# SAIC-MONTREAL/multimodal-dynamics

Hardware: AMD Instinct MI355X
Metric: visuotactile samples/sec (train) + ELBO vs CPU ref, cnn-mvae 64x64 bs256 @1/2/4/8 GPU (higher is better)
Workload: dtype f32x3; 1 GPU; cnn-mvae visuotactile+pose 64x64, bs=256 per GPU, fp32 storage and results, GEMMs in the fp32x3 arithmetic (exact three-term bf16 split of the fp32 operands, six of nine products on the bf16 matrix cores, fp32 accumulate; error vs fp64 <= native fp32 MFMA), seq_modeling train step (7 subset ELBOs + backward + Adam), BASELINE configs[1]; global_batch=256, parallelism=dp1, bn=local, launch=hip_graph

## Files before the change

include/mmdyn_hip.h:

```cpp
#ifndef MMDYN_HIP_H
#define MMDYN_HIP_H

#include <stdint.h>

#ifdef __cplusplus
extern "C" {
#endif

#define MMDYN_OK 0
#define MMDYN_ERR_SHAPE (-1)
#define MMDYN_ERR_NULL (-2)
#define MMDYN_ERR_RANGE (-3)

#define MMDYN_ACT_NONE 0
#define MMDYN_ACT_SWISH 1
#define MMDYN_ACT_RELU 2

#define MMDYN_DENSE 0
#define MMDYN_CONV 1
#define MMDYN_TCONV_S2P1 2
#define MMDYN_IM2COL3 3

#define MMDYN_TCONV_S1P0 4

// ... 273 lines not shown

int mmdyn_sgd_step(float* p, const float* g, float* momentum_buf, int64_t n, float lr, float momentum,
                   float weight_decay, float grad_scale, int first, void* stream);

int mmdyn_resize_ksize(int in_size, int out_size);
int mmdyn_resize_plan(int in_size, int out_size, int* bounds, int* coeffs);
int mmdyn_resize_u8_to_chw_f32(const uint8_t* src, const int* index, float* dst, int n_out, int Hin, int Win,
                               int Hout, int Wout, const int* xb, const int* xk, const int* yb, const int* yk,
                               void* stream);

int mmdyn_igemm_nt_mx(const void* A, const void* Bp, const float* bias, void* C, void* C_act, float* stats,
                      float* ws, const void* y, const float* mean, const float* rstd, const float* gamma,
                      const float* beta, int mode, int G, int Bg, int Hi, int Wi, int Cin, int Ho, int Wo, int N,
                      int ldc, int stride, int offset, int act, int splitk, int flags, uint32_t* arrival_flags, void* stream);
int mmdyn_wgrad_tn_mx(const void* D, const void* Gt, float* partial, int mode, int Bt, int Hr, int Wr, int Cd, int Hi,
                      int Wi, int Cg, int stride, int offset, int chunks, int flags, void* stream);
int mmdyn_split_planes(const float* x, void* planes, int64_t rows, int C, void* stream);
int mmdyn_igemm_planes_served(int mode, int G, int Bg, int Hi, int Wi, int Cin, int Ho, int Wo, int N);
int mmdyn_bn_swish_fwd_planes(const float* y, const float* mean, const float* rstd, const float* gamma, const float* beta,
                              float* a, void* a_planes, int G, int rows_per_group, int C, void* stream);
int mmdyn_bn_swish_bwd_apply_planes(const float* da, const float* y, const float* mean, const float* rstd, const float* gamma,
                                    const float* beta, const float* sums, float* dy, void* dy_planes, int G, int rows_per_group,
                                    int C, int da_is_du, void* stream);
int mmdyn_bn_eval_swish_bwd(const float* da, const float* y, const float* mean, const float* rstd, const float* gamma,
                            const float* beta, float* dy, void* dy_planes, float* partial, int G, int rows_per_group, int C,
                            int da_is_du, void* stream);
int mmdyn_bn_swish_fwd_b16(const uint16_t* y, const float* mean, const float* rstd, const float* gamma,
                           const float* beta, uint16_t* a, int G, int rows_per_group, int C, int half, void* stream);
int mmdyn_bn_swish_bwd_reduce_b16(const uint16_t* da, const uint16_t* y, const float* mean, const float* rstd,
                                  const float* gamma, const float* beta, float* partial, int G, int rows_per_group,
                                  int C, int half, void* stream);
int mmdyn_bn_swish_bwd_apply_b16(const uint16_t* da, const uint16_t* y, const float* mean, const float* rstd,
                                 const float* gamma, const float* beta, const float* sums, uint16_t* dy, int G,
                                 int rows_per_group, int C, int da_is_du, int half, void* stream);
int mmdyn_act_bwd_b16(const uint16_t* dh, const uint16_t* u, uint16_t* du, int64_t n, int act, int half, void* stream);
int mmdyn_tconv_out3_fwd_b16(const uint16_t* a, const float* w, float* out, int Bt, int Hi, int Wi, int half,
                             void* stream);

int mmdyn_nchw_to_nhwc(const float* in, float* out, int B, int C, int HW, void* stream);
int mmdyn_nhwc_to_nchw(const float* in, float* out, int B, int C, int HW, void* stream);

int mmdyn_concat_condition(const float* x, const float* cond, const int64_t* cond_idx, float* out, int* bad_index, int rows,
                           int K, int ldx, int cd, int width, void* stream);
int mmdyn_concat_condition_tiled(const float* x, const float* cond, const int64_t* cond_idx, float* out, int* bad_index, int rows,
                                 int x_rows, int K, int ldx, int cd, int width, void* stream);

// ... 5 lines not shown
```

multimodal-dynamics_amd/csrc/bn.hip:

```cpp
#include "common.h"

namespace {

static int tile_rows_for(int rows_per_group) {
  int t = rows_per_group / 256 / 32 * 32;
  return t < 32 ? 32 : (t > 512 ? 512 : t);
}

struct BnParams {
  const float* mean;
  const float* rstd;
  const float* gamma;
  const float* beta;
};

template <int MODE, typename TA>
__global__ __launch_bounds__(256) void colreduce_kernel(const TA* __restrict__ y,
                                                        const TA* __restrict__ da, BnParams bp,
                                                        float* __restrict__ partial, int rows_per_group,
                                                        int C, int T, int tile_rows) {
  __shared__ float red[256 * 8];
  const int tid = threadIdx.x;
  const int g = blockIdx.y, t = blockIdx.x;
  const int CV = C >> 2;
// ... 331 lines not shown
  for (int64_t i = blockIdx.x * (int64_t)blockDim.x + threadIdx.x; i < total8; i += (int64_t)gridDim.x * blockDim.x) {
    const int cv = (int)(i % CV);
    const int64_t row = i / CV;
    const int g = (int)(row / rows_per_group);
    f32x4 v[2], d[2], o[2];
    ldv_nt<float>(y + i * 8, v);
    ldv_nt<float>(y + i * 8 + 4, v + 1);
    ldv_nt<float>(da + i * 8, d);
    ldv_nt<float>(da + i * 8 + 4, d + 1);
#pragma unroll
    for (int q = 0; q < 2; ++q) {
      const int c0 = cv * 8 + q * 4;
      f32x4 m = *reinterpret_cast<const f32x4*>(bp.mean + (size_t)g * C + c0);
      f32x4 r = *reinterpret_cast<const f32x4*>(bp.rstd + (size_t)g * C + c0);
      f32x4 ga = *reinterpret_cast<const f32x4*>(bp.gamma + c0);
      f32x4 be = *reinterpret_cast<const f32x4*>(bp.beta + c0);
      f32x4 s0 = *reinterpret_cast<const f32x4*>(sums + ((size_t)g * 2 + 0) * C + c0);
      f32x4 s1 = *reinterpret_cast<const f32x4*>(sums + ((size_t)g * 2 + 1) * C + c0);
#pragma unroll
      for (int k = 0; k < 4; ++k) {
        float xh = (v[q][k] - m[k]) * r[k];
        float u = ga[k] * xh + be[k];
        float du = da_is_du ? d[q][k] : d[q][k] * swish_gradf_(u);
        o[q][k] = ga[k] * r[k] * (du - s0[k] * inv_n - xh * (s1[k] * inv_n));
      }
    }
    if (dy) {
      stv_nt<float>(dy + i * 8, o);
      stv_nt<float>(dy + i * 8 + 4, o + 1);
    }
    store_planes8(dyp + row * 3 * (int64_t)C + cv * 8, C, o[0], o[1]);
  }
}

template <bool NEED_Y, bool PARTIAL>
__global__ __launch_bounds__(256) void bn_eval_swish_bwd_kernel(const float* __restrict__ da, const float* __restrict__ y, BnParams bp,
                                                                float* __restrict__ dy, bf16_t* __restrict__ dyp,
                                                                float* __restrict__ partial, int rows_per_group, int C, int T,
                                                                int tile_rows, int da_is_du) {
  __shared__ float red[PARTIAL ? 256 * 16 : 1];
  const int tid = threadIdx.x;
  const int g = blockIdx.y, t = blockIdx.x;
  const int CV = C >> 3;
  const int RL = 256 / CV;
  const int rl = tid / CV, cv = tid - rl * CV;
  const int r_begin = t * tile_rows;
  const int r_end = min(rows_per_group, r_begin + tile_rows);
// ... 323 lines not shown
```

multimodal-dynamics_amd/csrc/common.h:

```cpp
#pragma once
#include <hip/hip_runtime.h>
#include <stdint.h>
#include <stdlib.h>
#include "mmdyn_hip.h"

typedef float f32x16 __attribute__((ext_vector_type(16)));
typedef float f32x4 __attribute__((ext_vector_type(4)));

typedef uint16_t bf16_t;
template <typename T> __device__ __forceinline__ f32x4 ld4(const T* p);
template <> __device__ __forceinline__ f32x4 ld4<float>(const float* p) { return *reinterpret_cast<const f32x4*>(p); }
template <> __device__ __forceinline__ f32x4 ld4<bf16_t>(const bf16_t* p) {
  const uint2 u = *reinterpret_cast<const uint2*>(p);
  f32x4 v;
  v[0] = __uint_as_float(u.x << 16);
  v[1] = __uint_as_float(u.x & 0xffff0000u);
  v[2] = __uint_as_float(u.y << 16);
  v[3] = __uint_as_float(u.y & 0xffff0000u);
  return v;
}
template <typename T> __device__ __forceinline__ float ld1(const T* p);
template <> __device__ __forceinline__ float ld1<float>(const float* p) { return *p; }
template <> __device__ __forceinline__ float ld1<bf16_t>(const bf16_t* p) { return __uint_as_float((uint32_t)*p << 16); }
__device__ __forceinline__ uint32_t pack2_bf16(float lo, float hi) {
// ... 228 lines not shown
  return v;
}

__device__ __forceinline__ void block_atomic_add(double v, double* dst, double scale = 1.0) {
  v = wave_sum_d(v);
  __shared__ double red[4];
  if ((threadIdx.x & 63) == 0) red[threadIdx.x >> 6] = v;
  __syncthreads();
  if (threadIdx.x == 0) atomicAdd(dst, scale * (red[0] + red[1] + red[2] + red[3]));
}

constexpr float POE_EPS = 1e-8f;

constexpr uint32_t ALL_PRESENT = 0x01010101u;
__device__ __forceinline__ bool has(uint32_t word, int m) { return ((word >> (8 * m)) & 0xffu) != 0u; }

__device__ __forceinline__ float sigmoid_exact(float v) { return 1.f / (1.f + expf(-v)); }
__device__ __forceinline__ float sigmoidf_(float x) { return __builtin_amdgcn_rcpf(1.0f + __expf(-x)); }
__device__ __forceinline__ float swishf_(float x) { return x * sigmoidf_(x); }
__device__ __forceinline__ float swish_gradf_(float x) {
  float s = sigmoidf_(x);
  return s * (1.0f + x * (1.0f - s));
}
__device__ __forceinline__ float apply_act(float x, int act) {
  if (act == MMDYN_ACT_SWISH) return swishf_(x);
  if (act == MMDYN_ACT_RELU) return x > 0.f ? x : 0.f;
  return x;
}
__device__ __forceinline__ float act_grad(float x, int act) {
  if (act == MMDYN_ACT_SWISH) return swish_gradf_(x);
  if (act == MMDYN_ACT_RELU) return x > 0.f ? 1.f : 0.f;
  return 1.f;
}

__device__ __forceinline__ void bce_elem(float x, float t, float& loss, float& sig) {
  const float e = __expf(-fabsf(x));
  const float inv = __frcp_rn(__fadd_rn(1.f, e));
  loss = __fadd_rn(__fsub_rn(fmaxf(x, 0.f), __fmul_rn(x, t)), __logf(__fadd_rn(1.f, e)));
  sig = x >= 0.f ? inv : __fmul_rn(e, inv);
}

int mmdyn_conv3_nt_try(const float* A, const float* Bp, const float* bias, void* C, void* C_act, float* stats, int G,
                       int Bg, int Hi, int Wi, int Ho, int Wo, int N, int ldc, int act, int splitk, const void* bn_y,
                       const float* bn_mean, const float* bn_rstd, const float* bn_gamma, const float* bn_beta,
                       int c_b16, int bny_b16, int b_b16, hipStream_t st);
int mmdyn_conv3_wgrad_try(const void* D, const float* Gt, float* partial, int Bt, int Hr, int Wr, int Cd, int Hi,
// ... 25 lines not shown
```

multimodal-dynamics_amd/csrc/conv3.hip:

```cpp
#include "common.h"

namespace {

struct Conv3Geom {
  int G, Bg, Hi, Wi, Ho, ldc;
  int act, want_act_out, want_stats, w_b16;
  int tiles_per_group;
  const void* bn_y;
  const float* bn_mean;
  const float* bn_rstd;
  const float* bn_gamma;
  const float* bn_beta;
};

#define GLOBAL_AS __attribute__((address_space(1)))
typedef GLOBAL_AS char* gchar_p;
__device__ __forceinline__ gchar_p sgpr_ptr(const void* p) {
  const uint64_t u = reinterpret_cast<uint64_t>(p);
  const uint32_t lo = __builtin_amdgcn_readfirstlane((uint32_t)u), hi = __builtin_amdgcn_readfirstlane((uint32_t)(u >> 32));
  return (gchar_p)(((uint64_t)hi << 32) | lo);
}
template <typename T> __device__ __forceinline__ float gld1(gchar_p p);
template <> __device__ __forceinline__ float gld1<float>(gchar_p p) { return *(GLOBAL_AS const float*)p; }
template <> __device__ __forceinline__ float gld1<bf16_t>(gchar_p p) {
  return __uint_as_float((uint32_t)(*(GLOBAL_AS const bf16_t*)p) << 16);
}
template <> __device__ __forceinline__ float gld1<half_t>(gchar_p p) { return h2f(*(GLOBAL_AS const uint16_t*)p); }
template <typename T> struct store16 { typedef bf16_t type; };
template <> struct store16<half_t> { typedef half_t type; };

constexpr int C3_N = 32;
template <typename T, bool BN, int ACT, int SEGS>
__global__ __launch_bounds__(256) __attribute__((amdgpu_waves_per_eu(4, 4))) void conv3_nt_kernel(
    const float* __restrict__ img, const float* __restrict__ Wp, T* __restrict__ C, T* __restrict__ C_act,
    float* __restrict__ stats, const Conv3Geom g) {
  __shared__ float Ws[32 * 65];
  __shared__ float red[4][2][32];
  const int tid = threadIdx.x, lane = tid & 63;
  const int wave = __builtin_amdgcn_readfirstlane(tid >> 6);
  const int x = lane & 31, h = lane >> 5;
  for (int i = tid; i < 512; i += 256) {
    const f32x4 v = g.w_b16 == 2 ? ld4<half_t>(reinterpret_cast<const half_t*>(Wp) + 4 * i)
                    : g.w_b16 ? ld4<bf16_t>(reinterpret_cast<const bf16_t*>(Wp) + 4 * i)
                              : reinterpret_cast<const f32x4*>(Wp)[i];
    const int n = i >> 4, k = (i & 15) * 4;
    Ws[n * 65 + k + 0] = v[0];
    Ws[n * 65 + k + 1] = v[1];
    Ws[n * 65 + k + 2] = v[2];
    Ws[n * 65 + k + 3] = v[3];
  }
  __syncthreads();
  float bw[24];
  auto load_bw = [&]() {
#pragma unroll
    for (int j = 0; j < 24; ++j) bw[j] = Ws[x * 65 + (j >> 3) * 16 + ((j >> 1) & 3) * 4 + 2 * (j & 1) + h];
  };
  if (!BN) load_bw();

  const float bn_g = BN ? g.bn_gamma[x] : 0.f, bn_b = BN ? g.bn_beta[x] : 0.f;
  const int ntiles = g.G * g.tiles_per_group;

  constexpr int C3_HI = 64 * SEGS, C3_HO = 32 * SEGS;
  constexpr int UNITS = C3_HO * SEGS;
  int xl[2];
#pragma unroll
  for (int q = 0; q < 2; ++q) xl[q] = 2 * x - 1 + 2 * q + h;
  const unsigned voffB = (4 * h * C3_N + x) * sizeof(T);
  constexpr unsigned IMG_B = 3 * C3_HI * C3_HI * sizeof(float);
  constexpr unsigned OROW_B = 32 * C3_N * sizeof(T);

  struct TileAt {
    gchar_p imgb;
    size_t orow;
    int y, seg;
    unsigned xoB[2];
    bool xok[2];
  };
  auto locate = [&](int t) {
    TileAt p;
    const int u = t * 4 + wave;
    const int ib = u / UNITS, rem = u - ib * UNITS;
    p.y = rem / SEGS;
    p.seg = rem - p.y * SEGS;
    p.imgb = sgpr_ptr(reinterpret_cast<const char*>(img) + (size_t)ib * IMG_B + (size_t)p.seg * 256 - 4);
    p.orow = (size_t)u * OROW_B;
#pragma unroll
    for (int q = 0; q < 2; ++q) {
      p.xok[q] = (unsigned)(p.seg * 64 + xl[q]) < (unsigned)C3_HI;
      p.xoB[q] = (unsigned)((p.xok[q] ? xl[q] + 1 : 1) * 4);
    }
    return p;
  };
  auto load_a = [&](const TileAt& p, int j) {
    const int ci = j >> 3, yin = 2 * p.y - 1 + ((j >> 1) & 3);
    const bool yok = (unsigned)yin < (unsigned)C3_HI;
    const gchar_p rowp = p.imgb + (unsigned)((ci * C3_HI + (yok ? yin : 0)) * C3_HI) * 4u;
    return gld1<float>(rowp + p.xoB[j & 1]);
  };
  auto erow = [](int e) { return (unsigned)(((e & 3) + 8 * (e >> 2)) * C3_N * sizeof(T)); };

  float a[24], yv[16];
  int t = blockIdx.x;
  if (t >= ntiles) return;
  TileAt cur = locate(t);
#pragma unroll
  for (int j = 0; j < 24; ++j) a[j] = load_a(cur, j);
  if (BN) {
    const gchar_p yb = sgpr_ptr(reinterpret_cast<const char*>(g.bn_y) + cur.orow) + voffB;
#pragma unroll
    for (int e = 0; e < 16; ++e) yv[e] = gld1<T>(yb + erow(e));
  }
  for (; t < ntiles; t += gridDim.x) {
    const int tn = t + gridDim.x < ntiles ? t + gridDim.x : t;
    const TileAt nxt = locate(tn);
    const int grp = (BN || g.want_stats) ? __builtin_amdgcn_readfirstlane((t / (UNITS / 4)) / g.Bg) : 0;
    if (BN) load_bw();
    float bn_m = 0.f, bn_r = 0.f;
    if (BN) {
      bn_m = g.bn_mean[grp * 32 + x];
      bn_r = g.bn_rstd[grp * 32 + x];
    }
    f32x16 acc;
#pragma unroll
    for (int e = 0; e < 16; ++e) acc[e] = 0.f;
#pragma unroll
    for (int j = 0; j < 24; ++j) {
      const int yin = 2 * cur.y - 1 + ((j >> 1) & 3);
      const bool ok = ((unsigned)yin < (unsigned)C3_HI) & cur.xok[j & 1];
      acc = __builtin_amdgcn_mfma_f32_32x32x2f32(ok ? a[j] : 0.f, bw[j], acc, 0, 0, 0);
      a[j] = load_a(nxt, j);
    }

    const gchar_p cb = sgpr_ptr(reinterpret_cast<const char*>(C) + cur.orow) + voffB;
    const gchar_p ab = sgpr_ptr(reinterpret_cast<const char*>(C_act) + cur.orow) + voffB;
    const gchar_p yb = sgpr_ptr(reinterpret_cast<const char*>(g.bn_y) + nxt.orow) + voffB;
    float cs = 0.f, cq = 0.f;
#pragma unroll
    for (int e = 0; e < 16; ++e) {
      float v = acc[e];
      if (BN) {
        const float xh = (yv[e] - bn_m) * bn_r;
        yv[e] = gld1<T>(yb + erow(e));
        v *= swish_gradf_(bn_g * xh + bn_b);
        cs += v;
        cq += v * xh;
      } else {
        cs += v;
        cq += v * v;
      }
      if (sizeof(T) == 2) {
        const float vn = __shfl_down(v, 1, 64);
        if (!(x & 1)) {
          *(GLOBAL_AS uint32_t*)(cb + erow(e)) = pack2<typename store16<T>::type>(v, vn);
          if (ACT >= 0)
            *(GLOBAL_AS uint32_t*)(ab + erow(e)) = pack2<typename store16<T>::type>(apply_act(v, ACT), apply_act(vn, ACT));
        }
      } else {
        *(GLOBAL_AS float*)(cb + erow(e)) = v;
        if (ACT >= 0) *(GLOBAL_AS float*)(ab + erow(e)) = apply_act(v, ACT);
      }
    }
    if (g.want_stats) {
      cs += __shfl_xor(cs, 32, 64);
      cq += __shfl_xor(cq, 32, 64);
      if (h == 0) {
        red[wave][0][x] = cs;
        red[wave][1][x] = cq;
      }
      __syncthreads();
      if (tid < 32) {
        float s0 = 0.f, q0 = 0.f;
#pragma unroll
        for (int w = 0; w < 4; ++w) {
// ... 192 lines not shown
      if (segs == 1) CONV3_LAUNCH(half_t, BN_, ACT_, 1);                                                           \
      else if (segs == 2) CONV3_LAUNCH(half_t, BN_, ACT_, 2);                                                      \
      else CONV3_LAUNCH(half_t, BN_, ACT_, 4);                                                                     \
    } else if (c_b16) {                                                                                            \
      if (segs == 1) CONV3_LAUNCH(bf16_t, BN_, ACT_, 1);                                                           \
      else if (segs == 2) CONV3_LAUNCH(bf16_t, BN_, ACT_, 2);                                                      \
      else CONV3_LAUNCH(bf16_t, BN_, ACT_, 4);                                                                     \
    } else {                                                                                                       \
      if (segs == 1) CONV3_LAUNCH(float, BN_, ACT_, 1);                                                            \
      else if (segs == 2) CONV3_LAUNCH(float, BN_, ACT_, 2);                                                       \
      else CONV3_LAUNCH(float, BN_, ACT_, 4);                                                                      \
    }                                                                                                              \
  }
  CONV3_CASE(4, true, -1)
  CONV3_CASE(-1, false, -1)
  CONV3_CASE(MMDYN_ACT_NONE, false, MMDYN_ACT_NONE)
  CONV3_CASE(MMDYN_ACT_SWISH, false, MMDYN_ACT_SWISH)
  CONV3_CASE(MMDYN_ACT_RELU, false, MMDYN_ACT_RELU)
#undef CONV3_LAUNCH
#undef CONV3_CASE
  MMDYN_LAUNCH_CHECK();
}

int mmdyn_conv3_wgrad_try(const void* D, const float* Gt, float* partial, int Bt, int Hr, int Wr, int Cd, int Hi,
                          int Wi, int Cg, int chunks, int d_b16, hipStream_t st, const float* bn_mean, const float* bn_rstd,
                          const float* bn_gamma, const float* bn_beta, int Bg) {
  if (Cd != 32 || Cg != 64 || Wr != Hr || Wi != Hi || Hi != 2 * Hr || (Hi != 64 && Hi != 128 && Hi != 256)) return 1;
  const int segs = Hi / 64;
  if ((int64_t)Bt * Hr * segs >= (1LL << 30)) return 1;
  Conv3WgradGeom g{};
  g.Bt = Bt;
  g.Hr = Hr;
  g.Hi = Hi;
  g.Wi = Wi;
  g.img_rows = Bt * Hr * segs;
  g.rows_per_chunk = ceil_div(g.img_rows, chunks);
  g.bn_mean = bn_mean;
  g.bn_rstd = bn_rstd;
  g.bn_gamma = bn_gamma;
  g.bn_beta = bn_beta;
  g.Bg = Bg > 0 ? Bg : Bt;
#define CONV3_WG(T_, S_)                                                                                                  \
  do {                                                                                                                    \
    if (bn_mean)                                                                                                          \
      hipLaunchKernelGGL((conv3_wgrad_kernel<T_, S_, true>), dim3(chunks), dim3(256), 0, st, (const T_*)D, Gt, partial, g); \
    else                                                                                                                  \
// ... 19 lines not shown
```

multimodal-dynamics_amd/mmdyn_hip/_lib.py:

```python
import ctypes
import os

_HERE = os.path.dirname(os.path.abspath(__file__))
LIB_PATH = os.environ.get("MMDYN_HIP_LIB") or os.path.join(_HERE, "libmmdyn_hip.so")

_P, _I, _L, _F, _Q = ctypes.c_void_p, ctypes.c_int, ctypes.c_int64, ctypes.c_float, ctypes.c_uint64


class PassExperts(ctypes.Structure):
    _fields_ = [("mu", _P * 4), ("lv", _P * 4), ("dmu", _P * 4), ("dlv", _P * 4), ("ld", _I * 4), ("dz", _P * 3),
                ("zdst", _P * 3), ("zpl", _P * 3)]


class PackEntry(ctypes.Structure):
    _fields_ = [("src", _P), ("dst", _P), ("kind", _I), ("rows_in", _I), ("cols_in", _I), ("rows_out", _I),
                ("cols_out", _I), ("ld_out", _I), ("dst_bf16", _I)]


class FeedGroups(ctypes.Structure):
    _fields_ = [("recon", _P * 4), ("obs", _P * 4), ("out", _P * 4), ("row_len", _I * 4), ("logits", _I * 4), ("column", _I * 4)]


class GatherGroups(ctypes.Structure):
    _fields_ = [("src", _P * 4), ("out", _P * 4), ("row_len", _I * 4), ("logits", _I * 4)]
# ... 68 lines not shown
    "mmdyn_cast_f32_to_bf16": "pp" + "l" + "p",
    "mmdyn_cast_bf16_to_f32": "pp" + "l" + "p",
    "mmdyn_linear_small_fwd": "pppp" + "iiii" + "p",
    "mmdyn_linear_small_bwd": "pppppp" + "iii" + "f" + "p",
    "mmdyn_poe_fwd": "pppppp" + "iiii" + "p",
    "mmdyn_poe_bwd": "ppppppp" + "f" + "iiii" + "pp",
    "mmdyn_reparam_fwd": "ppppp" + "iii" + "p",
    "mmdyn_reparam_bwd": "pppp" + "f" + "pp" + "iii" + "p",
    "mmdyn_bce_logits": "ppppp" + "l" + "iii" + "f" + "p",
    "mmdyn_bce_logits_groups": "ppppp" + "i" + "l" + "f" + "p",
    "mmdyn_bce_logits_groups_masked": "ppppppp" + "i" + "l" + "iii" + "f" + "p",
    "mmdyn_mse": "pppp" + "l" + "f" + "p",
    "mmdyn_mse_groups": "ppppp" + "i" + "l" + "f" + "p",
    "mmdyn_elbo_assemble": "ppppp" + "ii" + "ff" + "pp",
    "mmdyn_adam_step": "ppppp" + "l" + "fffff" + "p",
    "mmdyn_adam_step_guarded": "ppppp" + "l" + "fffff" + "p",
    "mmdyn_sgd_step": "ppp" + "l" + "ffff" + "i" + "p",
    "mmdyn_igemm_nt_mx": "pppppppppppp" + "iiiiiiiiiiiiii" + "i" + "pp",
    "mmdyn_wgrad_tn_mx": "ppp" + "iiiiiiiiiii" + "i" + "p",
    "mmdyn_split_planes": "pp" + "l" + "i" + "p",
    "mmdyn_igemm_planes_served": "iiiiiiiii",
    "mmdyn_bn_swish_fwd_planes": "ppppppp" + "iii" + "p",
    "mmdyn_bn_swish_bwd_apply_planes": "ppppppppp" + "iiii" + "p",
    "mmdyn_bn_eval_swish_bwd": "ppppppppp" + "iiii" + "p",
    "mmdyn_bn_swish_fwd_b16": "pppppp" + "iiii" + "p",
    "mmdyn_bn_swish_bwd_reduce_b16": "ppppppp" + "iiii" + "p",
    "mmdyn_bn_swish_bwd_apply_b16": "pppppppp" + "iiiii" + "p",
    "mmdyn_act_bwd_b16": "ppp" + "l" + "ii" + "p",
    "mmdyn_tconv_out3_fwd_b16": "ppp" + "iiii" + "p",
    "mmdyn_resize_ksize": "ii",
    "mmdyn_resize_plan": "ii" + "pp",
    "mmdyn_resize_u8_to_chw_f32": "ppp" + "iiiii" + "pppp" + "p",
    "mmdyn_nchw_to_nhwc": "pp" + "iii" + "p",
    "mmdyn_nhwc_to_nchw": "pp" + "iii" + "p",
    "mmdyn_tconv_out3_bn_bce_rows": "ppppppp" + "i" + "pp" + "i" + "ppp" + "iiiiii" + "p",
    "mmdyn_bce_logits_rows_groups": "ppp" + "i" + "ppp" + "iiiii" + "p",
    "mmdyn_mse_rows_groups": "pppp" + "iiii" + "p",
    "mmdyn_kl_rows": "ppp" + "iii" + "p",
    "mmdyn_elbo_assemble_rows": "pppppp" + "ii" + "ff" + "p" + "i" + "p",
    "mmdyn_concat_condition": "ppppp" + "iiiii" + "p",
    "mmdyn_poe_fwd_avail": "ppppppp" + "iiii" + "p",
    "mmdyn_poe_bwd_avail": "pppppppp" + "f" + "iiii" + "pp",
    "mmdyn_complete_select": "ppp" + "i" + "p" + "iii" + "p",
    "mmdyn_elbo_assemble_rows_avail": "ppppppppp" + "ii" + "ff" + "p" + "i" + "p",
    "mmdyn_tconv_out3_bn_bce_rows_grad": "ppppppp" + "i" + "pp" + "i" + "ppppp" + "i" + "f" + "iiiii" + "p",
    "mmdyn_bce_logits_rows_groups_grad": "ppp" + "i" + "ppppp" + "i" + "f" + "iiii" + "p",
# ... 61 lines not shown
```

multimodal-dynamics_amd/mmdyn_hip/layers.py:

```python
import weakref

import torch

from . import ops
from .ops import ACT_NONE, ACT_SWISH, ACT_RELU, DENSE, CONV, TCONV_S2P1, IM2COL3, TCONV_S1P0
from .models.shapes import BN_EPS, BN_MOMENTUM, FEAT


def _new(like, *shape, dtype=torch.float32):
    if isinstance(like, ops.Planes):
        like = like.t
    return torch.empty(shape, device=like.device, dtype=dtype)


ACT_DTYPE = torch.float32
W_DTYPE = torch.float32


def _act(like, *shape):
    return torch.empty(shape, device=like.device, dtype=ACT_DTYPE)


def _cdiv(a, b):
    return (a + b - 1) // b
# ... 31 lines not shown
        ops.B.igemm_nt(A, Bp, None, C, None, None, ws, DENSE, 1, rows, 1, 1, K, 1, 1, N, N, 1, 0, ACT_NONE, splitk)
        ops.B.splitk_reduce(ws, bias, C, Ca, splitk, rows, N, act)
    else:
        ops.B.igemm_nt(A, Bp, bias, C, Ca, None, None, DENSE, 1, rows, 1, 1, K, 1, 1, N, N, 1, 0, act, 1)
    return C, Ca


PLANES = True
PLANE_TWIN = {}


def _plane_twin(Wp):
    ent = PLANE_TWIN.get(Wp.data_ptr())
    if ent is None:
        return None
    if ent[0]() is not Wp:
        if ent[0]() is None:
            del PLANE_TWIN[Wp.data_ptr()]
        return None
    return ent[1]


PATCH_PLANES = True


def planes_served(mode, G, Bg, Hi, Cin, Ho, N):
    served = getattr(ops.B, "igemm_planes_served", None) if PLANES else None
    if N == 32 and not PATCH_PLANES:
        return False
    return bool(served is not None and ACT_DTYPE == torch.float32 and served(mode, G, Bg, Hi, Hi, Cin, Ho, Ho, N))


def split_operands(x, Wp, mode, G, Bg, Hi, Cin, Ho, N):
    if isinstance(Wp, ops.Planes):
        return x, Wp
    xin = x.t if isinstance(x, ops.Planes) else x
    if xin.dtype not in (torch.float32, torch.bfloat16) or Wp.dtype != torch.float32 or not planes_served(mode, G, Bg, Hi, Cin, Ho, N):
        if isinstance(x, ops.Planes):
            raise ValueError("mmdyn_hip: a plane operand for a launch the plane-ring kernel does not serve")
        return x, Wp
    if not isinstance(x, ops.Planes):
        xp = ops.Planes(x.numel() // Cin, Cin, x.device)
        ops.B.split_planes(x, xp)
        x = xp
    wp = _plane_twin(Wp)
    if wp is None or wp.C != Cin or wp.rows * Cin != Wp.numel():
# ... 177 lines not shown
        ops.backend_op("bn_eval_swish_bwd")(da, y, mean, rstd, bn.gamma, bn.beta, dy, partial, G, rows_per_group, C, False, planes=dyp)
        if partial is not None:
            _bn_eval_param_grads(y, partial, T, dgamma, dbeta, G, C)
        return dy if dyp is None else dyp
    partial = _new(y, G, T, 2, C)
    ops.B.bn_swish_bwd_reduce(da, y, mean, rstd, bn.gamma, bn.beta, partial, G, rows_per_group, C)
    sums = _bn_backward_sums(y, partial, T, dgamma, dbeta, G, C)
    dy, dyp = _apply_out(y, planes_out)
    if dyp is not None:
        ops.B.bn_swish_bwd_apply(da, y, mean, rstd, bn.gamma, bn.beta, sums, None, G, rows_per_group, C, planes=dyp)
        return dyp
    ops.B.bn_swish_bwd_apply(da, y, mean, rstd, bn.gamma, bn.beta, sums, dy, G, rows_per_group, C)
    return dy


def dgrad_bn_swish_backward(x, Wp, mode, G, Bg, Hi, Cin, Ho, N, stride, offset, y, mean, rstd, bn, dgamma, dbeta, planes_out=False,
                            eval_mode=False):
    rows_per_group = Bg * Ho * Ho
    if eval_mode:
        _eval_mode_check()
    if y.dtype == torch.float32 and mode != IM2COL3:
        x, Wp = split_operands(x, Wp, mode, G, Bg, Hi, Cin, Ho, N)
    T = _stat_tiles(x, Wp, mode, G, Bg, Hi, Cin, Ho, N)
    du = torch.empty_like(y)
    partial = _new(y, G, T, 2, N)
    ops.B.igemm_nt_dgrad_bn(x, Wp, du, partial, y, mean, rstd, bn.gamma, bn.beta, mode, G, Bg, Hi, Hi, Cin, Ho, Ho, N,
                            stride, offset)
    if eval_mode:
        if dgamma is not None or dbeta is not None:
            _bn_eval_param_grads(y, partial, T, dgamma, dbeta, G, N)
        dy, dyp = _apply_out(y, planes_out)
        ops.backend_op("bn_eval_swish_bwd")(du, None, mean, rstd, bn.gamma, bn.beta, dy, None, G, rows_per_group, N, True, planes=dyp)
        return dy if dyp is None else dyp
    sums = _bn_backward_sums(y, partial, T, dgamma, dbeta, G, N)
    dy, dyp = _apply_out(y, planes_out)
    if dyp is not None:
        ops.B.bn_swish_bwd_apply(du, y, mean, rstd, bn.gamma, bn.beta, sums, None, G, rows_per_group, N, True, planes=dyp)
        return dyp
    ops.B.bn_swish_bwd_apply(du, y, mean, rstd, bn.gamma, bn.beta, sums, dy, G, rows_per_group, N, True)
    return dy


def wgrad(D, Gt, canon, mode, Bt, Hr, Cd, Hi, Cg, stride=1, offset=0, cg_canon=None, perm=0, defer=None):
    if defer is not None:
        defer.append((D, Gt, canon, mode, Bt, Hr, Cd, Hi, Cg, stride, offset, cg_canon, perm))
        return
    rows = Bt * Hr * Hr
    taps = 16 if mode == CONV else 1
# ... 347 lines not shown
            with ctx():
                try:
                    next(gen)
                except StopIteration as e:
                    results[i] = e.value
                    live.remove(i)
    return results


def encoder_trunk_forward(*a, **k):
    return run(encoder_trunk_forward_steps(*a, **k))


def encoder_trunk_forward_steps(P, buf, x, G=1, repeat=1, packed=None, training=True):
    Bt = x.shape[0]
    Bg = Bt // G
    convs, S = enc_layout(P)
    if tuple(x.shape[1:]) != (3, S, S):
        raise ValueError(f"mmdyn_hip: this encoder takes [B,3,{S},{S}] images, got {tuple(x.shape)}")
    pk = packed if packed is not None else pack_now(encoder_pack_specs(P))
    c = {"Bt": Bt, "G": G, "Bg": Bg, "pk": pk, "S": S, "training": bool(training)}
    H = S // 2
    W1p = pk["W1p"]
    u1, a1 = _act(x, Bt * H * H, 32), _act(x, Bt * H * H, 32)
    ops.B.igemm_nt(x, W1p, None, u1, a1, None, None, IM2COL3, 1, Bt, S, S, 64, H, H, 32, 32, 1, 0,
                   ACT_SWISH, 1)
    yield
    stages, a, cin = [], a1, 32
    if len(convs) and planes_served(CONV, G, Bg, H, 32, H // 2, P[f"conv_net.{convs[0]}.weight"].shape[0]):
        a = as_planes(a1, 32)
    for j, i in enumerate(convs):
        cout = P[f"conv_net.{i}.weight"].shape[0]
        last = j == len(convs) - 1
        Ho, stride, offset = (H - 3, 1, 0) if last else (H // 2, 2, -1)
        bn = _bn_of(P, buf, f"conv_net.{i + 1}")
        y, st, T = conv_like(a, pk[f"W{j + 2}k"], CONV, G, Bg, H, cin, Ho, cout, stride, offset, training)
        want = False
        if not last:
            nlast = j + 1 == len(convs) - 1
            want = planes_served(CONV, G, Bg, Ho, cout, Ho - 3 if nlast else Ho // 2, P[f"conv_net.{convs[j + 1]}.weight"].shape[0])
        an, m, r = bn_swish_from_partials(y, st, T, bn, G, Bg * Ho * Ho, cout, repeat, planes=want)
        stages.append(dict(i=i, Hi=H, Ho=Ho, cin=cin, cout=cout, stride=stride, offset=offset, a_in=a, y=y, a=an, m=m, r=r,
                           bn=bn))
        a, cin, H = an, cout, Ho
        yield
    u5, h = dense(a, pk["Wf"], P["fc_net.0.bias"], Bt, FEAT, 512, ACT_SWISH, want_act=True)
    c.update(x=x, u1=u1, a1=a1, u5=u5, stages=stages)
    return h, c


def encoder_trunk_backward(*a, **k):
    return run(encoder_trunk_backward_steps(*a, **k))
# ... 306 lines not shown
```

multimodal-dynamics_amd/mmdyn_hip/ops.py:

```python
import ctypes

import os

import torch

from . import _lib
from ._lib import PassExperts, FeedGroups, GatherGroups, EnsembleGroups, MAX_PASSES, MAX_EXPERTS, FEED_GROUPS, check

ACT_NONE, ACT_SWISH, ACT_RELU = 0, 1, 2
DENSE, CONV, TCONV_S2P1, IM2COL3, TCONV_S1P0 = 0, 1, 2, 3, 4
ROW_GROUPS_MAX = 8
PLAN_TOP_MAX = 8
REFIT_N_MAX = 4096


def _ptr(t, dtype=torch.float32):
    if t is None:
        return None
    if not t.is_cuda:
        raise RuntimeError("mmdyn_hip: the HIP path needs GPU tensors (got a CPU tensor); there is no CPU fallback")
    if t.dtype != dtype:
        raise TypeError(f"mmdyn_hip: expected {dtype}, got {t.dtype}")
    if not t.is_contiguous():
        raise ValueError("mmdyn_hip: tensor must be contiguous")
# ... 534 lines not shown
    def bn_bwd_finalize_sums(self, sums, sums_f, dgamma, dbeta, G, C, sums_scale, beta_acc):
        check(self.lib.mmdyn_bn_bwd_finalize_sums(_ptr(sums, torch.float64), _ptr(sums_f), _ptr(dgamma), _ptr(dbeta), G, C,
                                                  float(sums_scale), float(beta_acc), _stream()),
              "mmdyn_bn_bwd_finalize_sums")

    def bn_swish_bwd_apply(self, da, y, mean, rstd, gamma, beta, sums, dy, G, rows_per_group, C, da_is_du=False, planes=None):
        if planes is not None:
            if planes.rows != G * rows_per_group or planes.C != C:
                raise ValueError("mmdyn_hip: bn_swish_bwd_apply: plane tensor of the wrong shape")
            check(self.lib.mmdyn_bn_swish_bwd_apply_planes(_ptr(da), _ptr(y), _ptr(mean), _ptr(rstd), _ptr(gamma), _ptr(beta), _ptr(sums),
                                                           _ptr(dy), planes.t.data_ptr(), G, rows_per_group, C, int(da_is_du), _stream()),
                  "mmdyn_bn_swish_bwd_apply_planes")
            return
        (pd, d16), (py, y16), (po, o16) = _aptr(da), _aptr(y), _aptr(dy)
        if not (d16 == y16 == o16):
            raise TypeError("mmdyn_hip: bn_swish_bwd_apply tensors must share the storage type")
        if y16:
            check(self.lib.mmdyn_bn_swish_bwd_apply_b16(pd, py, _ptr(mean), _ptr(rstd), _ptr(gamma), _ptr(beta), _ptr(sums), po,
                                                        G, rows_per_group, C, int(da_is_du), _half(y16), _stream()),
                  "mmdyn_bn_swish_bwd_apply_b16")
            return
        check(self.lib.mmdyn_bn_swish_bwd_apply(pd, py, _ptr(mean), _ptr(rstd), _ptr(gamma), _ptr(beta), _ptr(sums), po, G,
                                                rows_per_group, C, int(da_is_du), _stream()), "mmdyn_bn_swish_bwd_apply")

    def bn_eval_swish_bwd(self, da, y, mean, rstd, gamma, beta, dy, partial, G, rows_per_group, C, da_is_du=False, planes=None):
        if planes is not None and (planes.rows != G * rows_per_group or planes.C != C):
            raise ValueError("mmdyn_hip: bn_eval_swish_bwd: plane tensor of the wrong shape")
        n = G * rows_per_group * C
        for t in (da, y, dy):
            if t is not None and t.numel() != n:
                raise ValueError("mmdyn_hip: bn_eval_swish_bwd: da / y / dy must hold G * rows_per_group * C elements")
        if partial is not None and partial.numel() != G * self.colstats_tiles(rows_per_group) * 2 * C:
            raise ValueError("mmdyn_hip: bn_eval_swish_bwd: partial must be [G][colstats_tiles(rows_per_group)][2][C]")
        if mean.numel() != G * C or rstd.numel() != G * C or gamma.numel() != C or beta.numel() != C:
            raise ValueError("mmdyn_hip: bn_eval_swish_bwd: mean / rstd are [G][C], gamma / beta [C]")
        check(self.lib.mmdyn_bn_eval_swish_bwd(_ptr(da), _ptr(y), _ptr(mean), _ptr(rstd), _ptr(gamma), _ptr(beta), _ptr(dy),
                                               None if planes is None else planes.t.data_ptr(), _ptr(partial), G, rows_per_group, C,
                                               int(da_is_du), _stream()), "mmdyn_bn_eval_swish_bwd")

    def act_fwd(self, u, h, act):
        check(self.lib.mmdyn_act_fwd(_ptr(u), _ptr(h), u.numel(), act, _stream()), "mmdyn_act_fwd")

    def act_bwd(self, dh, u, du, act):
        (pd, d16), (pu, u16), (po, o16) = _aptr(dh), _aptr(u), _aptr(du)
        if not (d16 == u16 == o16):
            raise TypeError("mmdyn_hip: act_bwd tensors must share the storage type")
# ... 694 lines not shown
```

multimodal-dynamics_amd/mmdyn_hip/profiling.py:

```python
import collections

import torch

from . import ops

PAD_CYCLES = 100000
HOST_ONLY = {"igemm_stat_tiles", "colstats_tiles", "wgrad_chunks", "igemm_planes_served"}


def _canon(name, a):
    if name == "igemm_nt_dgrad_bn":
        A, Bp, C, stats, y, mean, rstd, gamma, beta, mode, G, Bg, Hi, Wi, Cin, Ho, Wo, N, stride, offset = a
        name, a = "igemm_nt", (A, Bp, y, C, None, stats, None, mode, G, Bg, Hi, Wi, Cin, Ho, Wo, N, N, stride, offset, 0, 1)
    if name == "igemm_nt_dgrad_act":
        A, Bp, C, u, act, mode, G, Bg, Hi, Wi, Cin, Ho, Wo, N, stride, offset = a
        name, a = "igemm_nt", (A, Bp, u, C, None, None, None, mode, G, Bg, Hi, Wi, Cin, Ho, Wo, N, N, stride, offset, 0, 1)
    if name == "igemm_nt_grouped":
        A, Bp, bias, C, C_act, u, G, rows, K, N, act = a
        name, a = "igemm_nt", (A, Bp, bias if u is None else u, C, C_act, None, None, ops.DENSE, G, rows, 1, 1, K, 1, 1, N, N, 1, 0, act, 1)
    if name == "wgrad_tn_grouped":
        D, Gt, partial, G, rows, Cd, Cg, chunks = a
        name, a = "wgrad_tn", (D, Gt, partial, ops.DENSE, G * rows, 1, 1, Cd, 1, 1, Cg, 1, 0, chunks)
    if name == "wgrad_out3_bn":
        y, mean, rstd, gamma, beta, Gt, partial, G, Bg, Hr, chunks = a
        return "conv3_wgrad", (y, Gt, partial, ops.IM2COL3, G * Bg, Hr, Hr, 32, 2 * Hr, 2 * Hr, 64, 1, 0, chunks)
    if name == "tconv_out3_bn_fwd":
        return "tconv_out3_fwd", a
    if name == "igemm_nt" and a[7] == ops.IM2COL3 and a[10] in (64, 128, 256) and \
            tuple(a[10:17]) == (a[10], a[10], 64, a[10] // 2, a[10] // 2, 32, 32):
        return "conv3_nt", a
    if name == "igemm_nt" and a[7] == ops.TCONV_S2P1 and tuple(a[10:16]) in ((16, 16, 64, 32, 32, 32), (32, 32, 32, 64, 64, 32),
                                                                            (64, 64, 32, 128, 128, 32)) and \
            getattr(ops.B, "precision", "fp32") == "fp32" and all(not torch.is_tensor(t) or t.dtype == torch.float32 for t in a[:4]):
        return "tconv_patch", a
    if name == "wgrad_tn" and a[3] == ops.IM2COL3 and a[8] in (64, 128, 256) and \
            tuple(a[5:11]) == (a[8] // 2, a[8] // 2, 32, a[8], a[8], 64):
        return "conv3_wgrad", a
    return name, a


def _flops(name, a):
    if name in ("igemm_nt", "conv3_nt", "tconv_patch"):
        (mode, G, Bg, Hi, Wi, Cin, Ho, Wo, N) = a[7:16]
        if mode == ops.DENSE:
            return 2.0 * G * Bg * Ho * Wo * N * Cin
        if mode == ops.CONV:
            return 2.0 * G * Bg * Ho * Wo * N * 16 * Cin
        if mode == ops.TCONV_S1P0:
            return 2.0 * G * Bg * Hi * Wi * N * 16 * Cin
        if mode == ops.IM2COL3:
# ... 93 lines not shown
```

Before: 54320 samples/s.

## Fuse split-plane output into first conv3 forward and BN-backward dgrad

The first 3-channel conv's forward kernel now writes the activation straight into the three-term bf16 plane layout, which removes a separate as_planes conversion pass and the fp32 activation buffer. For the BN-backward through the conv3 output layer, the dgrad GEMM runs twice: once for the column statistics and once to apply the BN backward and emit dy planes. This avoids materialising the full fp32 du tensor and the separate apply kernel. It spends an extra recompute of the small conv3 GEMM, and pins the FMA contraction order so the fused and unfused paths round the same way.

```diff
diff --git a/include/mmdyn_hip.h b/include/mmdyn_hip.h
--- a/include/mmdyn_hip.h
+++ b/include/mmdyn_hip.h
@@ -319,6 +319,13 @@
 int mmdyn_bn_swish_bwd_apply_planes(const float* da, const float* y, const float* mean, const float* rstd, const float* gamma,
                                     const float* beta, const float* sums, float* dy, void* dy_planes, int G, int rows_per_group,
                                     int C, int da_is_du, void* stream);
+int mmdyn_conv3_fwd_planes(const float* x, const float* Wp, float* C, void* act_planes, int G, int Bg, int H, int act,
+                           void* stream);
+int mmdyn_conv3_dgrad_bn_stats(const float* dlogits, const float* Wp, float* stats, const float* y, const float* mean,
+                               const float* rstd, const float* gamma, const float* beta, int G, int Bg, int H, void* stream);
+int mmdyn_conv3_dgrad_bn_apply_planes(const float* dlogits, const float* Wp, const float* y, const float* mean,
+                                      const float* rstd, const float* gamma, const float* beta, const float* sums,
+                                      void* dy_planes, int G, int Bg, int H, void* stream);
 int mmdyn_bn_eval_swish_bwd(const float* da, const float* y, const float* mean, const float* rstd, const float* gamma,
                             const float* beta, float* dy, void* dy_planes, float* partial, int G, int rows_per_group, int C,
                             int da_is_du, void* stream);
diff --git a/multimodal-dynamics_amd/csrc/bn.hip b/multimodal-dynamics_amd/csrc/bn.hip
--- a/multimodal-dynamics_amd/csrc/bn.hip
+++ b/multimodal-dynamics_amd/csrc/bn.hip
@@ -377,7 +377,7 @@
         float xh = (v[q][k] - m[k]) * r[k];
         float u = ga[k] * xh + be[k];
         float du = da_is_du ? d[q][k] : d[q][k] * swish_gradf_(u);
-        o[q][k] = ga[k] * r[k] * (du - s0[k] * inv_n - xh * (s1[k] * inv_n));
+        o[q][k] = bn_swish_bwd_dy(du, xh, ga[k], r[k], s0[k], s1[k], inv_n, q == 1 && k == 3);
       }
     }
     if (dy) {
diff --git a/multimodal-dynamics_amd/csrc/common.h b/multimodal-dynamics_amd/csrc/common.h
--- a/multimodal-dynamics_amd/csrc/common.h
+++ b/multimodal-dynamics_amd/csrc/common.h
@@ -274,6 +274,14 @@
   float s = sigmoidf_(x);
   return s * (1.0f + x * (1.0f - s));
 }
+__device__ __forceinline__ float bn_swish_bwd_dy(float du, float xh, float ga, float r, float s0, float s1, float inv_n,
+                                                 bool tail_fused) {
+#pragma clang fp contract(off)
+  const float t0 = __builtin_fmaf(-inv_n, s0, du);
+  const float s1n = inv_n * s1;
+  const float t = tail_fused ? __builtin_fmaf(-s1n, xh, t0) : t0 - s1n * xh;
+  return (ga * r) * t;
+}
 __device__ __forceinline__ float apply_act(float x, int act) {
   if (act == MMDYN_ACT_SWISH) return swishf_(x);
   if (act == MMDYN_ACT_RELU) return x > 0.f ? x : 0.f;
diff --git a/multimodal-dynamics_amd/csrc/conv3.hip b/multimodal-dynamics_amd/csrc/conv3.hip
--- a/multimodal-dynamics_amd/csrc/conv3.hip
+++ b/multimodal-dynamics_amd/csrc/conv3.hip
@@ -11,6 +11,9 @@
   const float* bn_rstd;
   const float* bn_gamma;
   const float* bn_beta;
+  bf16_t* planes;
+  const float* bn_sums;
+  float inv_n;
 };
 
 #define GLOBAL_AS __attribute__((address_space(1)))
@@ -29,8 +32,14 @@
 template <typename T> struct store16 { typedef bf16_t type; };
 template <> struct store16<half_t> { typedef half_t type; };
 
+__device__ __forceinline__ void stat_acc_as_stored(float du, float xh, float& cs, float& cq) {
+#pragma clang fp contract(off)
+  cs = cs + du;
+  cq = __builtin_fmaf(du, xh, cq);
+}
 constexpr int C3_N = 32;
-template <typename T, bool BN, int ACT, int SEGS>
+constexpr int C3_ROWS = 0, C3_ACT_PLANES = 1, C3_STATS = 2, C3_DY_PLANES = 3;
+template <typename T, bool BN, int ACT, int SEGS, int OUT = C3_ROWS>
 __global__ __launch_bounds__(256) __attribute__((amdgpu_waves_per_eu(4, 4))) void conv3_nt_kernel(
     const float* __restrict__ img, const float* __restrict__ Wp, T* __restrict__ C, T* __restrict__ C_act,
     float* __restrict__ stats, const Conv3Geom g) {
@@ -68,6 +77,11 @@
   const unsigned voffB = (4 * h * C3_N + x) * sizeof(T);
   constexpr unsigned IMG_B = 3 * C3_HI * C3_HI * sizeof(float);
   constexpr unsigned OROW_B = 32 * C3_N * sizeof(T);
+  constexpr bool PLANES = OUT == C3_ACT_PLANES || OUT == C3_DY_PLANES;
+  static_assert(OUT == C3_ROWS || sizeof(T) == 4, "the plane-row and statistics-only forms are fp32 storage only");
+  static_assert(BN == (OUT == C3_STATS || OUT == C3_DY_PLANES) || OUT == C3_ROWS, "C3_STATS / C3_DY_PLANES belong to the BN epilogue");
+  constexpr unsigned PROW_B = 3 * C3_N * sizeof(bf16_t);
+  const unsigned voffP = (4 * h + (x & 1)) * PROW_B + (x & ~1) * sizeof(bf16_t);
 
   struct TileAt {
     gchar_p imgb;
@@ -98,6 +112,7 @@
     return gld1<float>(rowp + p.xoB[j & 1]);
   };
   auto erow = [](int e) { return (unsigned)(((e & 3) + 8 * (e >> 2)) * C3_N * sizeof(T)); };
+  auto prow = [](int e) { return (unsigned)(((e & 3) + 8 * (e >> 2)) * PROW_B); };
 
   float a[24], yv[16];
   int t = blockIdx.x;
@@ -134,21 +149,48 @@
     const gchar_p cb = sgpr_ptr(reinterpret_cast<const char*>(C) + cur.orow) + voffB;
     const gchar_p ab = sgpr_ptr(reinterpret_cast<const char*>(C_act) + cur.orow) + voffB;
     const gchar_p yb = sgpr_ptr(reinterpret_cast<const char*>(g.bn_y) + nxt.orow) + voffB;
-    float cs = 0.f, cq = 0.f;
+    const gchar_p pb = sgpr_ptr(reinterpret_cast<const char*>(g.planes) + (PLANES ? cur.orow / 2 * 3 : 0)) + voffP;
+    float ap_s0 = 0.f, ap_s1 = 0.f;
+    if (OUT == C3_DY_PLANES) {
+      ap_s0 = g.bn_sums[(grp * 2 + 0) * 32 + x];
+      ap_s1 = g.bn_sums[(grp * 2 + 1) * 32 + x];
+    }
+    float cs = 0.f, cq = 0.f, pv = 0.f;
 #pragma unroll
     for (int e = 0; e < 16; ++e) {
       float v = acc[e];
+      float o = 0.f;
       if (BN) {
         const float xh = (yv[e] - bn_m) * bn_r;
         yv[e] = gld1<T>(yb + erow(e));
         v *= swish_gradf_(bn_g * xh + bn_b);
-        cs += v;
-        cq += v * xh;
+        if (OUT == C3_DY_PLANES) {
+          o = bn_swish_bwd_dy(v, xh, bn_g, bn_r, ap_s0, ap_s1, g.inv_n, (x & 7) == 7);
+        } else if (OUT == C3_STATS) {
+          stat_acc_as_stored(v, xh, cs, cq);
+        } else {
+          cs += v;
+          cq += v * xh;
+        }
       } else {
         cs += v;
         cq += v * v;
+        if (OUT == C3_ACT_PLANES) o = apply_act(v, ACT);
       }
-      if (sizeof(T) == 2) {
+      if (PLANES) {
+        if (OUT == C3_ACT_PLANES) *(GLOBAL_AS float*)(cb + erow(e)) = v;
+        if (!(e & 1)) {
+          pv = o;
+        } else {
+          const float got = __shfl_xor((x & 1) ? pv : o, 1, 64);
+          uint32_t p_hi, p_mid, p_lo;
+          split3_bf16((x & 1) ? got : pv, (x & 1) ? o : got, p_hi, p_mid, p_lo);
+          *(GLOBAL_AS uint32_t*)(pb + prow(e - 1)) = p_hi;
+          *(GLOBAL_AS uint32_t*)(pb + prow(e - 1) + 64) = p_mid;
+          *(GLOBAL_AS uint32_t*)(pb + prow(e - 1) + 128) = p_lo;
+        }
+      } else if (OUT == C3_STATS) {
+      } else if (sizeof(T) == 2) {
         const float vn = __shfl_down(v, 1, 64);
         if (!(x & 1)) {
           *(GLOBAL_AS uint32_t*)(cb + erow(e)) = pack2<typename store16<T>::type>(v, vn);
@@ -387,6 +429,70 @@
   MMDYN_LAUNCH_CHECK();
 }
 
+namespace {
+int conv3_planes_launch(int out, const float* img, const float* Wp, float* C, float* stats, void* planes, const float* y,
+                        const float* mean, const float* rstd, const float* gamma, const float* beta, const float* sums, int G,
+                        int Bg, int H, int act, hipStream_t st) {
+  if (G <= 0 || Bg <= 0 || H != 64) return MMDYN_ERR_SHAPE;
+  const int Ho = H / 2;
+  if ((int64_t)G * Bg * Ho * Ho * C3_N >= (1LL << 31)) return MMDYN_ERR_RANGE;
+  Conv3Geom g{};
+  g.G = G;
+  g.Bg = Bg;
+  g.Hi = H;
+  g.Wi = H;
+  g.Ho = Ho;
+  g.ldc = C3_N;
+  g.act = act;
+  g.want_stats = stats != nullptr;
+  g.tiles_per_group = Bg * Ho * Ho / 128;
+  g.bn_y = y;
+  g.bn_mean = mean;
+  g.bn_rstd = rstd;
+  g.bn_gamma = gamma;
+  g.bn_beta = beta;
+  g.planes = reinterpret_cast<bf16_t*>(planes);
+  g.bn_sums = sums;
+  g.inv_n = 1.f / (float)(Bg * Ho * Ho);
+  const int ntiles = G * g.tiles_per_group;
+  const dim3 grid(ntiles < CONV3_GRID ? ntiles : CONV3_GRID);
+  float* none = nullptr;
+#define CONV3_PLANES(BN_, ACT_, OUT_) \
+  hipLaunchKernelGGL((conv3_nt_kernel<float, BN_, ACT_, 1, OUT_>), grid, dim3(256), 0, st, img, Wp, C, none, stats, g)
+  if (out == C3_STATS) CONV3_PLANES(true, -1, C3_STATS);
+  else if (out == C3_DY_PLANES) CONV3_PLANES(true, -1, C3_DY_PLANES);
+  else if (act == MMDYN_ACT_SWISH) CONV3_PLANES(false, MMDYN_ACT_SWISH, C3_ACT_PLANES);
+  else if (act == MMDYN_ACT_RELU) CONV3_PLANES(false, MMDYN_ACT_RELU, C3_ACT_PLANES);
+  else if (act == MMDYN_ACT_NONE) CONV3_PLANES(false, MMDYN_ACT_NONE, C3_ACT_PLANES);
+  else return MMDYN_ERR_SHAPE;
+#undef CONV3_PLANES
+  MMDYN_LAUNCH_CHECK();
+}
+}
+
+extern "C" int mmdyn_conv3_fwd_planes(const float* x, const float* Wp, float* C, void* act_planes, int G, int Bg, int H, int act,
+                                      void* stream) {
+  if (!x || !Wp || !C || !act_planes) return MMDYN_ERR_NULL;
+  return conv3_planes_launch(C3_ACT_PLANES, x, Wp, C, nullptr, act_planes, nullptr, nullptr, nullptr, nullptr, nullptr, nullptr, G,
+                             Bg, H, act, (hipStream_t)stream);
+}
+
+extern "C" int mmdyn_conv3_dgrad_bn_stats(const float* dlogits, const float* Wp, float* stats, const float* y, const float* mean,
+                                          const float* rstd, const float* gamma, const float* beta, int G, int Bg, int H,
+                                          void* stream) {
+  if (!dlogits || !Wp || !stats || !y || !mean || !rstd || !gamma || !beta) return MMDYN_ERR_NULL;
+  return conv3_planes_launch(C3_STATS, dlogits, Wp, nullptr, stats, nullptr, y, mean, rstd, gamma, beta, nullptr, G, Bg, H,
+                             MMDYN_ACT_NONE, (hipStream_t)stream);
+}
+
+extern "C" int mmdyn_conv3_dgrad_bn_apply_planes(const float* dlogits, const float* Wp, const float* y, const float* mean,
+                                                 const float* rstd, const float* gamma, const float* beta, const float* sums,
+                                                 void* dy_planes, int G, int Bg, int H, void* stream) {
+  if (!dlogits || !Wp || !y || !mean || !rstd || !gamma || !beta || !sums || !dy_planes) return MMDYN_ERR_NULL;
+  return conv3_planes_launch(C3_DY_PLANES, dlogits, Wp, nullptr, nullptr, dy_planes, y, mean, rstd, gamma, beta, sums, G, Bg, H,
+                             MMDYN_ACT_NONE, (hipStream_t)stream);
+}
+
 int mmdyn_conv3_wgrad_try(const void* D, const float* Gt, float* partial, int Bt, int Hr, int Wr, int Cd, int Hi,
                           int Wi, int Cg, int chunks, int d_b16, hipStream_t st, const float* bn_mean, const float* bn_rstd,
                           const float* bn_gamma, const float* bn_beta, int Bg) {
diff --git a/multimodal-dynamics_amd/mmdyn_hip/_lib.py b/multimodal-dynamics_amd/mmdyn_hip/_lib.py
--- a/multimodal-dynamics_amd/mmdyn_hip/_lib.py
+++ b/multimodal-dynamics_amd/mmdyn_hip/_lib.py
@@ -114,6 +114,9 @@
     "mmdyn_igemm_planes_served": "iiiiiiiii",
     "mmdyn_bn_swish_fwd_planes": "ppppppp" + "iii" + "p",
     "mmdyn_bn_swish_bwd_apply_planes": "ppppppppp" + "iiii" + "p",
+    "mmdyn_conv3_fwd_planes": "pppp" + "iiii" + "p",
+    "mmdyn_conv3_dgrad_bn_stats": "pppppppp" + "iii" + "p",
+    "mmdyn_conv3_dgrad_bn_apply_planes": "ppppppppp" + "iii" + "p",
     "mmdyn_bn_eval_swish_bwd": "ppppppppp" + "iiii" + "p",
     "mmdyn_bn_swish_fwd_b16": "pppppp" + "iiii" + "p",
     "mmdyn_bn_swish_bwd_reduce_b16": "ppppppp" + "iiii" + "p",
diff --git a/multimodal-dynamics_amd/mmdyn_hip/layers.py b/multimodal-dynamics_amd/mmdyn_hip/layers.py
--- a/multimodal-dynamics_amd/mmdyn_hip/layers.py
+++ b/multimodal-dynamics_amd/mmdyn_hip/layers.py
@@ -77,6 +77,14 @@
 
 
 PATCH_PLANES = True
+CONV1_PLANES = True
+OUT3_RECOMPUTE = True
+
+
+def _conv3_plane_op(name, switch, S, *tensors):
+    if not switch or S != 64 or ACT_DTYPE != torch.float32 or any(t.dtype != torch.float32 for t in tensors):
+        return None
+    return getattr(ops.B, name, None)
 
 
 def planes_served(mode, G, Bg, Hi, Cin, Ho, N):
@@ -300,8 +308,17 @@
     if y.dtype == torch.float32 and mode != IM2COL3:
         x, Wp = split_operands(x, Wp, mode, G, Bg, Hi, Cin, Ho, N)
     T = _stat_tiles(x, Wp, mode, G, Bg, Hi, Cin, Ho, N)
+    partial = _new(y, G, T, 2, N)
+    if mode == IM2COL3 and not eval_mode and planes_out:
+        stats_op = _conv3_plane_op("conv3_dgrad_bn_stats", OUT3_RECOMPUTE, Hi, x, Wp, y)
+        apply_op = _conv3_plane_op("conv3_dgrad_bn_apply_planes", OUT3_RECOMPUTE, Hi, x, Wp, y)
+        if stats_op is not None and apply_op is not None:
+            stats_op(x, Wp, partial, y, mean, rstd, bn.gamma, bn.beta, G, Bg, Hi)
+            sums = _bn_backward_sums(y, partial, T, dgamma, dbeta, G, N)
+            dyp = ops.Planes(y.shape[0], y.shape[1], y.device)
+            apply_op(x, Wp, y, mean, rstd, bn.gamma, bn.beta, sums, dyp, G, Bg, Hi)
+            return dyp
     du = torch.empty_like(y)
-    partial = _new(y, G, T, 2, N)
     ops.B.igemm_nt_dgrad_bn(x, Wp, du, partial, y, mean, rstd, bn.gamma, bn.beta, mode, G, Bg, Hi, Hi, Cin, Ho, Ho, N,
                             stride, offset)
     if eval_mode:
@@ -695,12 +712,20 @@
     c = {"Bt": Bt, "G": G, "Bg": Bg, "pk": pk, "S": S, "training": bool(training)}
     H = S // 2
     W1p = pk["W1p"]
-    u1, a1 = _act(x, Bt * H * H, 32), _act(x, Bt * H * H, 32)
-    ops.B.igemm_nt(x, W1p, None, u1, a1, None, None, IM2COL3, 1, Bt, S, S, 64, H, H, 32, 32, 1, 0,
-                   ACT_SWISH, 1)
+    a_planes = bool(len(convs)) and planes_served(CONV, G, Bg, H, 32, H // 2, P[f"conv_net.{convs[0]}.weight"].shape[0])
+    u1 = _act(x, Bt * H * H, 32)
+    fwd_planes = _conv3_plane_op("conv3_fwd_planes", CONV1_PLANES and a_planes, S, x, W1p, u1)
+    if fwd_planes is not None:
+        a1, a = None, ops.Planes(Bt * H * H, 32, x.device)
+        fwd_planes(x, W1p, u1, a, 1, Bt, S, ACT_SWISH)
+    else:
+        a1 = _act(x, Bt * H * H, 32)
+        ops.B.igemm_nt(x, W1p, None, u1, a1, None, None, IM2COL3, 1, Bt, S, S, 64, H, H, 32, 32, 1, 0,
+                       ACT_SWISH, 1)
+        a = a1
     yield
-    stages, a, cin = [], a1, 32
-    if len(convs) and planes_served(CONV, G, Bg, H, 32, H // 2, P[f"conv_net.{convs[0]}.weight"].shape[0]):
+    stages, cin = [], 32
+    if a_planes and fwd_planes is None:
         a = as_planes(a1, 32)
     for j, i in enumerate(convs):
         cout = P[f"conv_net.{i}.weight"].shape[0]
diff --git a/multimodal-dynamics_amd/mmdyn_hip/ops.py b/multimodal-dynamics_amd/mmdyn_hip/ops.py
--- a/multimodal-dynamics_amd/mmdyn_hip/ops.py
+++ b/multimodal-dynamics_amd/mmdyn_hip/ops.py
@@ -580,6 +580,39 @@
             return
         check(self.lib.mmdyn_bn_swish_bwd_apply(pd, py, _ptr(mean), _ptr(rstd), _ptr(gamma), _ptr(beta), _ptr(sums), po, G,
                                                 rows_per_group, C, int(da_is_du), _stream()), "mmdyn_bn_swish_bwd_apply")
+
+    @staticmethod
+    def _conv3_shapes(name, img, Wp, G, Bg, H, **rows32):
+        rows = G * Bg * (H // 2) ** 2
+        if img.numel() != G * Bg * 3 * H * H or Wp.numel() != 32 * 64:
+            raise ValueError(f"mmdyn_hip: {name}: image / packed weight of the wrong shape")
+        for k, t in rows32.items():
+            if isinstance(t, Planes):
+                if t.rows != rows or t.C != 32 or not t.t.is_cuda or not t.t.is_contiguous():
+                    raise ValueError(f"mmdyn_hip: {name}: {k} must be a contiguous GPU plane tensor of [{rows}][3][32]")
+            elif t.numel() != rows * 32:
+                raise ValueError(f"mmdyn_hip: {name}: {k} must hold [{rows}][32] elements")
+
+    def conv3_fwd_planes(self, x, Wp, C, act_planes, G, Bg, H, act):
+        self._conv3_shapes("conv3_fwd_planes", x, Wp, G, Bg, H, C=C, act_planes=act_planes)
+        check(self.lib.mmdyn_conv3_fwd_planes(_ptr(x), _ptr(Wp), _ptr(C), act_planes.t.data_ptr(), G, Bg, H, int(act), _stream()),
+              "mmdyn_conv3_fwd_planes")
+
+    def conv3_dgrad_bn_stats(self, dlogits, Wp, stats, y, mean, rstd, gamma, beta, G, Bg, H):
+        self._conv3_shapes("conv3_dgrad_bn_stats", dlogits, Wp, G, Bg, H, y=y)
+        self._check_stat_tiles(stats, False, IM2COL3, G, Bg, H, H, 64, H // 2, H // 2, 32)
+        if mean.numel() != G * 32 or rstd.numel() != G * 32 or gamma.numel() != 32 or beta.numel() != 32:
+            raise ValueError("mmdyn_hip: conv3_dgrad_bn_stats: BatchNorm vectors of the wrong shape")
+        check(self.lib.mmdyn_conv3_dgrad_bn_stats(_ptr(dlogits), _ptr(Wp), _ptr(stats), _ptr(y), _ptr(mean), _ptr(rstd), _ptr(gamma),
+                                                  _ptr(beta), G, Bg, H, _stream()), "mmdyn_conv3_dgrad_bn_stats")
+
+    def conv3_dgrad_bn_apply_planes(self, dlogits, Wp, y, mean, rstd, gamma, beta, sums, dy_planes, G, Bg, H):
+        self._conv3_shapes("conv3_dgrad_bn_apply_planes", dlogits, Wp, G, Bg, H, y=y, dy_planes=dy_planes)
+        if mean.numel() != G * 32 or rstd.numel() != G * 32 or gamma.numel() != 32 or beta.numel() != 32 or sums.numel() != G * 64:
+            raise ValueError("mmdyn_hip: conv3_dgrad_bn_apply_planes: BatchNorm vectors / sums of the wrong shape")
+        check(self.lib.mmdyn_conv3_dgrad_bn_apply_planes(_ptr(dlogits), _ptr(Wp), _ptr(y), _ptr(mean), _ptr(rstd), _ptr(gamma),
+                                                         _ptr(beta), _ptr(sums), dy_planes.t.data_ptr(), G, Bg, H, _stream()),
+              "mmdyn_conv3_dgrad_bn_apply_planes")
 
     def bn_eval_swish_bwd(self, da, y, mean, rstd, gamma, beta, dy, partial, G, rows_per_group, C, da_is_du=False, planes=None):
         if planes is not None and (planes.rows != G * rows_per_group or planes.C != C):
diff --git a/multimodal-dynamics_amd/mmdyn_hip/profiling.py b/multimodal-dynamics_amd/mmdyn_hip/profiling.py
--- a/multimodal-dynamics_amd/mmdyn_hip/profiling.py
+++ b/multimodal-dynamics_amd/mmdyn_hip/profiling.py
@@ -26,6 +26,15 @@
         return "conv3_wgrad", (y, Gt, partial, ops.IM2COL3, G * Bg, Hr, Hr, 32, 2 * Hr, 2 * Hr, 64, 1, 0, chunks)
     if name == "tconv_out3_bn_fwd":
         return "tconv_out3_fwd", a
+    if name == "conv3_fwd_planes":
+        x, Wp, C, planes, G, Bg, H, act = a
+        return "conv3_nt", (x, Wp, None, C, planes, None, None, ops.IM2COL3, G, Bg, H, H, 64, H // 2, H // 2, 32, 32, 1, 0, act, 1)
+    if name == "conv3_dgrad_bn_stats":
+        x, Wp, stats, y, mean, rstd, gamma, beta, G, Bg, H = a
+        return "conv3_nt", (x, Wp, y, None, None, stats, None, ops.IM2COL3, G, Bg, H, H, 64, H // 2, H // 2, 32, 32, 1, 0, 0, 1)
+    if name == "conv3_dgrad_bn_apply_planes":
+        x, Wp, y, mean, rstd, gamma, beta, sums, planes, G, Bg, H = a
+        return "conv3_nt", (x, Wp, y, planes, None, None, None, ops.IM2COL3, G, Bg, H, H, 64, H // 2, H // 2, 32, 32, 1, 0, 0, 1)
     if name == "igemm_nt" and a[7] == ops.IM2COL3 and a[10] in (64, 128, 256) and \
             tuple(a[10:17]) == (a[10], a[10], 64, a[10] // 2, a[10] // 2, 32, 32):
         return "conv3_nt", a
```

Measured after the change: 55290 samples/s (median of 6 runs). 1.02x the previous value.
